# 30stomercury/Automatic-Speech-Recognition

Hardware: AMD Instinct MI355X
Metric: utterances/sec (train step) LibriSpeech-360 char-LAS @1/2/4/8 GPU; dev-clean WER (higher is better)
Workload: dtype bf16; 1 GPU; LibriSpeech-100 char LAS (BASELINE configs[1]): 3xpBLSTM-256 listener + 1xLSTM-512 speller, additive attention, MFCC-39, bucket B=48 T=1274, U=191, V=30; full train step fwd+bwd+clip+Adam; cell=lstm, per_gpu_batch=48, global_batch=48, frames=1274, dec_steps=191, parallelism=dp1, params=9679774

## Files before the change

automatic-speech-recognition_amd/csrc/las_common.h:

```cpp
#pragma once
#include <hip/hip_runtime.h>
#include <stdint.h>
#include <stddef.h>
#include "../../include/las_hip.h"

#if defined(__HIP_DEVICE_COMPILE__) && !defined(__gfx950__)
#error "liblas_hip.so is written for gfx950 (MI355X / CDNA4) only"
#endif

void las_set_error(const char* fmt, ...);
int las_device_cus();
int las_xcd_round_robin();

#define LAS_ARG(cond, ...)                                   \
    do { if (!(cond)) { las_set_error(__VA_ARGS__); return -1; } } while (0)
#define LAS_HIP(expr)                                        \
    do { hipError_t e__ = (expr);                            \
         if (e__ != hipSuccess) { las_set_error("%s -> %s", #expr, hipGetErrorString(e__)); \
                                  return (int)e__; } } while (0)
#ifdef LAS_DEBUG_SYNC
#define LAS_LAUNCHED()                                       \
    do { hipError_t e__ = hipGetLastError();                 \
         if (e__ == hipSuccess) e__ = hipDeviceSynchronize(); \
         if (e__ != hipSuccess) { las_set_error("%s:%d: launch failed: %s", __FILE__, __LINE__, hipGetErrorString(e__)); \
// ... 169 lines not shown
static inline int cdiv(long long a, long long b) { return (int)((a + b - 1) / b); }

extern "C" int las_colsum_dt(const void* X, int dtype, int rows, int cols, int ldx, float beta, float* out, void* ws,
                             size_t ws_bytes, void* stream);

size_t las_skinny_pack_bytes(int K, int N);
int las_skinny_pack(const float* W, int ldw, int K, int N, int transposed, void* packed, hipStream_t st);
int las_skinny_gemm(const float* A, int lda, int M, int K, const void* packed, int N, float* C, int ldc,
                    const float* bias, hipStream_t st);
int las_skinny_gemm_bf16(const unsigned short* A, int lda, int M, int K, const void* packed, int N, float* C, int ldc,
                         const float* bias, hipStream_t st);
int las_skinny_gemm_bf16_tanh(const unsigned short* A, int lda, int M, int K, const void* packed, int N, const float* bias, float* eh, int ldh,
                              unsigned short* b0, int ld0, unsigned short* b1, int ld1, hipStream_t st);
int las_skinny_gemm_bf16_tanh_bwd(const unsigned short* A, int lda, int M, int K, const void* packed, int N, float* C, int ldc, int c0, int D,
                                  const float* h, int ldh, const float* sa, int lda_, const float* sb, int ldb, int vlast, float* gp, int ldg,
                                  unsigned short* gb, int ldgb, hipStream_t st);
int las_skinny_gemm_bf16_lstm_bwd(const unsigned short* A, int lda, int M, int K, const void* packed, int N, float* C, int ldc, int c0, int D,
                                  const float* sa, int lda_, const float* sb, int ldb, int vlast, float* gp, int ldg, unsigned short* gb, int ldgb,
                                  const float* c, const float* cp, float* dC, int ldc_, hipStream_t st);
int las_skinny_lstm_bf16(const unsigned short* A, int lda, int M, int K, const void* packed, int D, const float* bias, float fb, const float* cprev,
                         float* c, float* h, float* gates, unsigned short* b0, int ld0, unsigned short* b1, int ld1, hipStream_t st);
bool las_skinny_ok(int M, int K, int N, int lda, const void* A);

typedef las_lstm_cell_args LstmCellLaunch;
int las_lstm_cell_rows_launch(const LstmCellLaunch& a, hipStream_t st);
int las_lstm_cell_check(const LstmCellLaunch& a);
int las_lstm_cell_rows_launch2(const LstmCellLaunch& a, const LstmCellLaunch& b, hipStream_t st);
```

automatic-speech-recognition_amd/csrc/speller.hip:

```cpp
#include "las_common.h"
#include "lstm_cell_rows.h"
#include <type_traits>
#include <math.h>

#define LAS_MAX_NL 4

constexpr int RNT = 1024;
constexpr int RNG = RNT / 32;
constexpr int RNW = RNT / 64;
constexpr int RNH = RNT / 128;

struct LoopProd {
    const u16x8_t* Bp; int KS, K, N, nct, M, pn, R;
    const float* bias;
    float* C; long long c_step; int ldc;
    unsigned long long* gA; int gA_row;
    unsigned long long* gC; int gC_row;
    unsigned long long* xcc;
    int nap;
    int budget;
    int* status;
};
#define LOOP_POLL_TIMEOUT(lp)                                                                                   \
    do { if ((lp).status) (lp).status[0] = LAS_SPELLER_STATUS_TIMEOUT; __builtin_amdgcn_s_waitcnt(0); __builtin_amdgcn_endpgm(); } while (0)
// ... 2578 lines not shown
}

__global__ __launch_bounds__(256) void dkeys_kernel(DecDev a, float* __restrict__ dKeys) {
    const int b = blockIdx.y, tt = blockIdx.x * 8 + (threadIdx.x >> 5), sl = threadIdx.x & 31;
    const int B = a.B, Tp = a.Tp, A = a.A, U = a.U;
    if (tt >= Tp) return;
    for (int a4 = sl; a4 < A / 4; a4 += 32) {
        const unsigned short* kr = a.keysbf + ((size_t)b * Tp + tt) * A + a4 * 4;
        const float k0 = bf2f(kr[0]), k1 = bf2f(kr[1]), k2 = bf2f(kr[2]), k3 = bf2f(kr[3]);
        float4 acc = make_float4(0.f, 0.f, 0.f, 0.f);
#pragma unroll 8
        for (int t = 0; t < U; ++t) {
            const float de = a.dE[((size_t)t * B + b) * Tp + tt];
            const float4 q4 = reinterpret_cast<const float4*>(a.Q + ((size_t)t * B + b) * A)[a4];
            const float v0 = tanh_fast(k0 + q4.x), v1 = tanh_fast(k1 + q4.y), v2 = tanh_fast(k2 + q4.z), v3 = tanh_fast(k3 + q4.w);
            acc.x = fmaf(de, 1.f - v0 * v0, acc.x); acc.y = fmaf(de, 1.f - v1 * v1, acc.y);
            acc.z = fmaf(de, 1.f - v2 * v2, acc.z); acc.w = fmaf(de, 1.f - v3 * v3, acc.w);
        }
        const float4 u4 = reinterpret_cast<const float4*>(a.u)[a4];
        float4* o = reinterpret_cast<float4*>(dKeys + ((size_t)b * Tp + tt) * A) + a4;
        float4 cur = *o;
        cur.x = fmaf(acc.x, u4.x, cur.x); cur.y = fmaf(acc.y, u4.y, cur.y); cur.z = fmaf(acc.z, u4.z, cur.z); cur.w = fmaf(acc.w, u4.w, cur.w);
        *o = cur;
    }
}

constexpr int EMB_MAX_V = 16384, EMB_MAX_N = 49152;
__global__ __launch_bounds__(1024) void emb_hist_kernel(const int* __restrict__ tok, int n, int V, int* __restrict__ start) {
    extern __shared__ int cnt[];
    int* part = cnt + V;
    const int tid = threadIdx.x;
    for (int v = tid; v < V; v += 1024) cnt[v] = 0;
    __syncthreads();
    for (int i = tid; i < n; i += 1024) { const int v = tok[i]; if (v >= 0 && v < V) atomicAdd(&cnt[v], 1); }
    __syncthreads();
    const int per = (V + 1023) / 1024, v0 = tid * per, v1 = min(V, v0 + per);
    int s_ = 0;
    for (int v = v0; v < v1; ++v) s_ += cnt[v];
    part[tid] = s_;
    __syncthreads();
    for (int off = 1; off < 1024; off <<= 1) {
        const int x = tid >= off ? part[tid - off] : 0;
        __syncthreads();
        part[tid] += x;
        __syncthreads();
    }
// ... 132 lines not shown
    w.fcS = o;    o += align256(C > 0 ? (size_t)U * B * Tp * C * f : 0);
    w.dfcS = o;   o += align256(C > 0 ? (size_t)U * B * Tp * C * f : 0);
    w.dlocwP = o; o += align256(C > 0 ? (size_t)B * DLW_SPLIT * Kc * C * f : 0);
    w.dlocbP = o; o += align256(C > 0 ? (size_t)B * DLW_SPLIT * C * f : 0);
    w.wide = o;   o += align256(wide_layout(B, Tp, A, D, NL, G, C).total);
    w.gemm = o;
    size_t big = (size_t)I0D * G * D;
    if ((size_t)D * V > big) big = (size_t)D * V;
    if ((size_t)8 * V * E > big) big = (size_t)8 * V * E;
    o += align256(big * 8 * f);
    w.total = o;
    return w;
}

static size_t act_save_f_offset(int U, int B, int Tp, int A) { return align256((size_t)LAS_ACT_HDR * 4 + (size_t)U * B * Tp * A * 2); }
extern "C" size_t las_speller_act_save_bytes(int U, int B, int Tp, int A, int C) {
    return act_save_f_offset(U, B, Tp, A) + (size_t)U * B * Tp * (C > 0 ? C : 0) * sizeof(float);
}
extern "C" size_t las_speller_workspace_bytes(int B, int Tp, int Hd, int A, int D, int NL, int E, int V, int U, int cell) {
    const int G = cell == LAS_CELL_LSTM ? 4 : 1;
    return bwd_layout(B, Tp, Hd, A, D, NL, E, V, U, G, 256, 16).total;
}

static int fill_dev(const las_speller_fwd_args* f, DecDev& d) {
    LAS_ARG(f, "speller: null args");
    LAS_ARG(f->B > 0 && f->Tp > 0 && f->Hd > 0 && f->A > 0 && f->D > 0 && f->E > 0 && f->V > 0 && f->U > 0,
            "speller: non-positive dimension");
    LAS_ARG(f->NL >= 1 && f->NL <= LAS_MAX_NL, "speller: NL=%d unsupported (1..%d)", f->NL, LAS_MAX_NL);
    LAS_ARG(f->D % 4 == 0 && f->Hd % 4 == 0, "speller: D and Hd must be multiples of 4");
    LAS_ARG(f->A % 4 == 0 && f->A <= 256, "speller: attention size must be a multiple of 4 and <= 256 (got %d)", f->A);
    LAS_ARG(f->cell == LAS_CELL_RNN || f->cell == LAS_CELL_LSTM, "speller: bad cell");
    LAS_ARG(f->mode == LAS_ATT_ADD || f->mode == LAS_ATT_LOC, "speller: bad attention mode");
    LAS_ARG(f->mode == LAS_ATT_ADD || (f->loc_w && f->loc_b && f->Wf && f->Kc > 0 && f->Kc <= 256 && f->C > 0 && f->C <= 16),
            "speller: location-aware attention needs loc_w/loc_b/Wf, Kc<=256, C<=16");
    LAS_ARG(f->enc && f->keys && f->enc_len && f->Ws && f->u && f->emb && f->Wv && f->bv && f->cellW && f->cellb,
            "speller: null parameter pointer");
    LAS_ARG(f->tokens_in && f->logits && f->alphas && f->hs && f->gates && f->xin0, "speller: null buffer pointer");
    LAS_ARG(f->cell == LAS_CELL_RNN || f->cs, "speller: lstm needs cs");
    LAS_ARG(!f->step_logits || f->tokens_out, "speller: step_logits needs tokens_out");
    LAS_ARG((((uintptr_t)f->keys | (uintptr_t)f->u | (uintptr_t)f->Ws) & 15) == 0, "speller: keys/u/Ws must be 16-byte aligned");
    d.B = f->B; d.Tp = f->Tp; d.Hd = f->Hd; d.A = f->A; d.D = f->D; d.NL = f->NL; d.E = f->E; d.V = f->V; d.U = f->U;
    d.mode = f->mode; d.Kc = f->mode == LAS_ATT_LOC ? f->Kc : 0; d.C = f->mode == LAS_ATT_LOC ? f->C : 0;
    d.step_logits = f->step_logits; d.flags = f->flags; d.fb = f->forget_bias; d.seed = f->seed;
    d.row_group = (f->row_group > 0 && f->B % f->row_group == 0) ? f->row_group : 0;
    d.shared_ops = ((f->flags & LAS_SPELLER_SHARED_OPERANDS) && d.row_group > 0) ? 1 : 0;
    LAS_ARG(!(f->flags & LAS_SPELLER_SHARED_OPERANDS) || d.row_group > 0, "speller: LAS_SPELLER_SHARED_OPERANDS needs row_group > 0 with B %% row_group == 0");
// ... 161 lines not shown
                if (int rc = f->companion ? las_lstm_cell_rows_launch2(c, *f->companion, st) : las_lstm_cell_rows_launch(c, st)) return rc;
                break;
            }
            if (skinny) {
                GEMM_OK(las_skinny_gemm_bf16(d.xbf, I0D, B, I0D, packF, GD, d.gates + ((size_t)0 * U + t) * B * GD, GD, f->cellb[0], st));
            } else {
                const bool hw = f->ws && f->ws_bytes > wl_.gemm;
                GEMM_OK(las_gemm(f->prec, 0, 0, B, GD, I0D, 1.f, d.xin0 + (size_t)t * B * I0D, I0D, 0, f->cellW[0], GD, 0, 0.f,
                                 d.gates + ((size_t)0 * U + t) * B * GD, GD, 0, f->cellb[0], LAS_ACT_NONE, 1, 0, 0,
                                 hw ? (char*)f->ws + wl_.gemm : nullptr, hw ? f->ws_bytes - wl_.gemm : 0, st));
            }
            for (int l = 1; l < NL; ++l) {
                hipLaunchKernelGGL((dec_pointwise_fwd_kernel<CELL, FAST>), dim3(B), dim3(256), 0, st, d, l - 1, t);
                LAS_LAUNCHED();
                float* gl = d.gates + ((size_t)l * U + t) * B * GD;
                GEMM_OK(las_gemm(f->prec, 0, 0, B, GD, D, 1.f, d.hs + ((size_t)(l - 1) * (U + 1) + t + 1) * B * D, D, 0,
                                 f->cellW[l], GD, 0, 0.f, gl, GD, 0, f->cellb[l], LAS_ACT_NONE, 1, 0, 0, nullptr, 0, st));
                GEMM_OK(las_gemm(f->prec, 0, 0, B, GD, D, 1.f, d.hs + ((size_t)l * (U + 1) + t) * B * D, D, 0,
                                 f->cellW[l] + (size_t)D * GD, GD, 0, 1.f, gl, GD, 0, nullptr, LAS_ACT_NONE, 1, 0, 0, nullptr, 0, st));
            }
        }
    }
    if (d.step_logits != 1) {
        GEMM_OK(las_gemm(f->prec, 0, 0, U * B, V, D, 1.f, d.hs + ((size_t)(NL - 1) * (U + 1) + 1) * B * D, D, 0, d.Wv, V, 0,
                         0.f, d.logits, V, 0, d.bv, LAS_ACT_NONE, 1, 0, 0, nullptr, 0, st));
    }
    return 0;
}

extern "C" int las_speller_fwd(const las_speller_fwd_args* f, void* stream) {
    DecDev d;
    if (int rc = fill_dev(f, d)) return rc;
    hipStream_t st = (hipStream_t)stream;
    const bool fast = f->prec == LAS_PREC_BF16;
    if (f->cell == LAS_CELL_LSTM)
        return fast ? speller_fwd_impl<LAS_CELL_LSTM, true>(f, d, st) : speller_fwd_impl<LAS_CELL_LSTM, false>(f, d, st);
    return fast ? speller_fwd_impl<LAS_CELL_RNN, true>(f, d, st) : speller_fwd_impl<LAS_CELL_RNN, false>(f, d, st);
}

template <int CELL, bool FAST>
static int speller_bwd_impl(const las_speller_bwd_args* bk, DecDev d, int part, hipStream_t st) {
    constexpr int G = CELL == LAS_CELL_LSTM ? 4 : 1;
    const las_speller_fwd_args* f = &bk->f;
    const int B = d.B, D = d.D, NL = d.NL, U = d.U, E = d.E, Hd = d.Hd, V = d.V, A = d.A, Tp = d.Tp;
    const int GD = G * D, I0D = E + Hd + D, TOP = NL - 1, prec = f->prec;
    const bool loc = d.mode == LAS_ATT_LOC;
    const BwdWs w = bwd_layout(B, Tp, Hd, A, D, NL, E, V, U, G, d.Kc, d.C);
    LAS_ARG(f->ws && f->ws_bytes >= w.total, "las_speller_bwd: workspace too small (%zu < %zu)", f->ws_bytes, w.total);
// ... 12 lines not shown
    if (p.lds_row > 64 * 1024) LAS_LDS_ATTR((dec_step_bwd_kernel<CELL, FAST, true>), 150 * 1024);
    const bool skinny = p.skinny, wide = p.family == LAS_SPELLER_RAN_WIDE, loop = p.family == LAS_SPELLER_RAN_LOOP;
    void* packB = base + w.packB;
    if (skinny) d.dgbf = (unsigned short*)(base + w.dgbf);
    if (p.family != LAS_SPELLER_RAN_F32_ROWS) {
        if ((part & 1) && p.bf_copies) GEMM_OK(make_bf_copies(d, base, w, st));
        d.dE = (float*)(base + w.dE);
    }
    if (part & 1) g_last_variant[1] = p.ran;
    if (p.act_save && bk->f.act_save) {
        d.actS = (unsigned*)bk->f.act_save;
        if (d.mode == LAS_ATT_LOC) d.fcSave = (float*)((char*)bk->f.act_save + act_save_f_offset(U, B, Tp, A));
    }
    if (skinny && (part & 1)) {
        if (loop) GEMM_OK(las_skinny_pack(f->cellW[0] + (size_t)E * GD, GD, GD, Hd + D, 1, packB, st));
        else      GEMM_OK(las_skinny_pack(f->cellW[0], GD, GD, I0D, 1, packB, st));
    }
    if (part & 1) {
    d.rec[0] = d.dXin0; d.recLd[0] = I0D; d.recOff[0] = E + Hd;
    for (int l = 1; l < NL; ++l) { d.rec[l] = tmp + (size_t)l * B * 2 * D; d.recLd[l] = 2 * D; d.recOff[l] = D; }

    LAS_HIP(hipMemsetAsync(base + w.dH, 0, w.dXin0 - w.dH, st));
    LAS_HIP(hipMemsetAsync(base + w.duRows, 0, w.dV - w.duRows, st));
    GEMM_OK(las_gemm(prec, 0, 1, U * B, D, V, 1.f, bk->dlogits, V, 0, d.Wv, V, 0, 0.f, dHl, D, 0, nullptr, LAS_ACT_NONE, 1, 0, 0,
                     nullptr, 0, st));
    for (int l = 0; l < NL; ++l)
        GEMM_OK(las_gemm(prec, 0, 0, U * B, A, D, 1.f, d.hs + (size_t)l * (U + 1) * B * D, D, 0, d.Ws + (size_t)l * D * A, A, 0,
                         l ? 1.f : 0.f, d.Q, A, 0, nullptr, LAS_ACT_NONE, 1, 0, 0, nullptr, 0, st));

    switch (p.family) {
    case LAS_SPELLER_RAN_LOOP:
        loop_prod_dims(d.lp, B, Hd + D, GD);
        d.lp.Bp = reinterpret_cast<const u16x8_t*>(packB); d.lp.bias = nullptr;
        d.lp.C = d.dXin0 + E; d.lp.c_step = (long long)B * I0D; d.lp.ldc = I0D;
        d.lp.gA = (unsigned long long*)(base + w.granG); d.lp.gA_row = GD / 4;
        d.lp.gC = (unsigned long long*)(base + w.granB); d.lp.gC_row = (Hd + D) / 2;
        d.lp.xcc = (unsigned long long*)(base + w.xccs);
        LAS_HIP(hipMemsetAsync(base + w.granG, 0, w.xccs + 256 * 8 - w.granG, st));
        GEMM_OK(with_ne(Tp, [&](auto ne) {
            constexpr int NE = decltype(ne)::value;
            if (p.locloop) LAS_LDS_LAUNCH((dec_loop_bwd_kernel<CELL, NE, true>), dim3(8 * (d.lp.pn + d.lp.R)), dim3(RNT), p.lds_loop, LOOP_LDS_MAX, st, d);
            else           LAS_LDS_LAUNCH((dec_loop_bwd_kernel<CELL, NE, false>), dim3(8 * (d.lp.pn + d.lp.R)), dim3(RNT), p.lds_loop, LOOP_LDS_MAX, st, d);
            return 0;
        }));
        break;
    case LAS_SPELLER_RAN_WIDE:
        GEMM_OK((wide_bwd_steps<CELL, FAST>(bk, d, w, base, packB, dHl, tmp, gws, gws_bytes, st)));
        break;
// ... 18 lines not shown
            if (t < 0) break;
            for (int l = TOP; l >= 0; --l) {
                const float* dG = d.gates + ((size_t)l * U + t) * B * GD;
                if (l == 0 && skinny) {
                    GEMM_OK(las_skinny_gemm_bf16(d.dgbf, GD, B, GD, packB, I0D, d.dXin0 + (size_t)t * B * I0D, I0D, nullptr, st));
                } else if (l == 0) {
                    GEMM_OK(las_gemm(prec, 0, 1, B, I0D, GD, 1.f, dG, GD, 0, f->cellW[0], GD, 0, 0.f, d.dXin0 + (size_t)t * B * I0D,
                                     I0D, 0, nullptr, LAS_ACT_NONE, 1, 0, 0, gws, gws_bytes, st));
                } else {
                    float* tl = tmp + (size_t)l * B * 2 * D;
                    GEMM_OK(las_gemm(prec, 0, 1, B, 2 * D, GD, 1.f, dG, GD, 0, f->cellW[l], GD, 0, 0.f, tl, 2 * D, 0, nullptr,
                                     LAS_ACT_NONE, 1, 0, 0, nullptr, 0, st));
                    hipLaunchKernelGGL((dec_pointwise_bwd_kernel<CELL, FAST>), dim3(B), dim3(256), 0, st, d, l - 1, t, (const float*)tl, 2 * D);
                    LAS_LAUNCHED();
                }
            }
        }
    }

    if (p.locloop) {
        hipLaunchKernelGGL(dkeys_loc_kernel, dim3(cdiv(Tp, 8), B), dim3(256), 0, st, d, bk->d_keys);
        LAS_LAUNCHED();
    } else if (!wide && p.family != LAS_SPELLER_RAN_F32_ROWS) {
        hipLaunchKernelGGL(dkeys_kernel, dim3(cdiv(Tp, 8), B), dim3(256), 0, st, d, bk->d_keys);
        LAS_LAUNCHED();
    }
    GEMM_OK(las_gemm(prec, 1, 0, Tp, Hd, U, 1.f, d.alphas, B * Tp, Tp, d.dXin0 + E, B * I0D, I0D, 1.f, bk->d_enc, Hd,
                     (long long)Tp * Hd, nullptr, LAS_ACT_NONE, B, 0, 0, nullptr, 0, st));
    }
    if (!(part & 2)) return 0;
    const int UB = U * B;
    GEMM_OK(las_gemm(prec, 1, 0, I0D, GD, UB, 1.f, d.xin0, I0D, 0, d.gates, GD, 0, 1.f, bk->dcellW[0], GD, 0, nullptr,
                     LAS_ACT_NONE, 1, 0, 0, gws, gws_bytes, st));
    for (int l = 0; l < NL; ++l) {
        const float* dG = d.gates + (size_t)l * U * B * GD;
        GEMM_OK(las_colsum(dG, UB, GD, GD, 1.f, bk->dcellb[l], gws, gws_bytes, st));
        if (l > 0) {
            GEMM_OK(las_gemm(prec, 1, 0, D, GD, UB, 1.f, d.hs + ((size_t)(l - 1) * (U + 1) + 1) * B * D, D, 0, dG, GD, 0, 1.f,
                             bk->dcellW[l], GD, 0, nullptr, LAS_ACT_NONE, 1, 0, 0, gws, gws_bytes, st));
            GEMM_OK(las_gemm(prec, 1, 0, D, GD, UB, 1.f, d.hs + (size_t)l * (U + 1) * B * D, D, 0, dG, GD, 0, 1.f,
                             bk->dcellW[l] + (size_t)D * GD, GD, 0, nullptr, LAS_ACT_NONE, 1, 0, 0, gws, gws_bytes, st));
        }
        GEMM_OK(las_gemm(prec, 1, 0, D, A, UB, 1.f, d.hs + (size_t)l * (U + 1) * B * D, D, 0, d.dQ, A, 0, 1.f,
                         bk->dWs + (size_t)l * D * A, A, 0, nullptr, LAS_ACT_NONE, 1, 0, 0, gws, gws_bytes, st));
    }
    GEMM_OK(las_gemm(prec, 1, 0, D, V, UB, 1.f, d.hs + ((size_t)TOP * (U + 1) + 1) * B * D, D, 0, bk->dlogits, V, 0, 1.f,
                     bk->dWv, V, 0, nullptr, LAS_ACT_NONE, 1, 0, 0, gws, gws_bytes, st));
// ... 70 lines not shown
```

automatic-speech-recognition_amd/las/_hip.py:

```python
import collections
import ctypes
import os
from ctypes import (POINTER, Structure, c_char_p, c_double, c_float, c_int, c_longlong, c_size_t,
                    c_void_p)

import torch

PREC_F32, PREC_BF16 = 0, 1
CELL_RNN, CELL_LSTM = 0, 1
ACT_NONE, ACT_TANH = 0, 1
ATT_ADD, ATT_LOC = 0, 1
DT_F32, DT_BF16 = 0, 1

_HERE = os.path.dirname(os.path.abspath(__file__))
LIB_PATH = os.environ.get("LAS_LIB_PATH") or os.path.join(os.path.dirname(_HERE), "lib", "liblas_hip.so")
_lib = None


class LstmCellArgs(Structure):
    _fields_ = [("x", c_void_p), ("x_bf16", c_int), ("ldx", c_int), ("I", c_int), ("ids", c_void_p), ("id_shift", c_int), ("xrows", c_void_p),
                ("h", c_void_p), ("ldh", c_int), ("Wx", c_void_p), ("Wh", c_void_p), ("bias", c_void_p), ("c_prev", c_void_p), ("fb", c_float),
                ("c_out", c_void_p), ("h_out", c_void_p), ("gates_out", c_void_p), ("M", c_int), ("H", c_int), ("fast", c_int),
                ("h_bf16", c_int), ("h_out_bf16", c_void_p)]

# ... 96 lines not shown
    "las_gemm_dt": (c_int, [c_int, c_int, c_int, c_int, c_int, c_int, c_float, c_void_p, c_int, c_longlong,
                            c_void_p, c_int, c_longlong, c_int, c_float, c_void_p, c_int, c_longlong, c_void_p, c_int,
                            c_int, c_int, c_int, c_void_p, c_size_t, c_void_p]),
    "las_gemm_workspace_bytes": (c_size_t, [c_int, c_int, c_int, c_int, c_int]),
    "las_wgrad_ih_hh_workspace_bytes": (c_size_t, [c_int, c_int, c_int, c_int, c_int, c_int]),
    "las_wgrad_ih_hh": (c_int, [c_void_p, c_void_p, c_int, c_int, c_void_p, c_int, c_longlong, c_void_p, c_int, c_int, c_int, c_int, c_int, c_int,
                                c_void_p, c_void_p, c_void_p, c_size_t, c_void_p]),
    "las_gemm_kk": (c_int, [c_int, c_int, c_int, c_void_p, c_longlong, c_void_p, c_longlong, c_void_p, c_int, c_longlong,
                            c_void_p, c_int, c_void_p]),
    "las_gemm_kk_tanhgrad": (c_int, [c_int, c_int, c_int, c_void_p, c_longlong, c_void_p, c_longlong, c_void_p, c_int, c_longlong,
                            c_void_p, c_int, c_void_p, c_longlong, c_void_p]),
    "las_colsum_workspace_bytes": (c_size_t, [c_int]),
    "las_colsum": (c_int, [c_void_p, c_int, c_int, c_int, c_float, c_void_p, c_void_p, c_size_t, c_void_p]),
    "las_tanh_bwd": (c_int, [c_void_p, c_int, c_void_p, c_int, c_void_p, c_int, c_int, c_int, c_void_p]),
    "las_rnn_seq_workspace_bytes": (c_size_t, [c_int, c_int, c_int, c_int]),
    "las_rnn_seq_io_dtype": (c_int, [c_int, c_int, c_int]),
    "las_rnn_seq_plan": (c_int, [c_int, c_int, c_int, c_int, c_int, c_int, c_int, POINTER(RnnSeqPlanInfo)]),
    "las_rnn_seq_fwd": (c_int, [POINTER(RnnSeqArgs), c_void_p]),
    "las_rnn_seq_bwd": (c_int, [POINTER(RnnSeqArgs), c_void_p]),
    "las_colsum_dt": (c_int, [c_void_p, c_int, c_int, c_int, c_int, c_float, c_void_p, c_void_p, c_size_t, c_void_p]),
    "las_tanh_bwd_dt": (c_int, [c_void_p, c_int, c_int, c_void_p, c_int, c_int, c_void_p, c_int, c_int, c_int, c_int, c_void_p]),
    "las_speller_workspace_bytes": (c_size_t, [c_int] * 10),
    "las_speller_act_save_bytes": (c_size_t, [c_int] * 5),
    "las_speller_fwd": (c_int, [POINTER(SpellerFwdArgs), c_void_p]),
    "las_speller_bwd": (c_int, [POINTER(SpellerBwdArgs), c_void_p]),
    "las_speller_bwd_part": (c_int, [POINTER(SpellerBwdArgs), c_int, c_void_p]),
    "las_speller_last_variant": (c_int, [c_int]),
    "las_bn_workspace_bytes": (c_size_t, [c_longlong, c_int]),
    "las_bn_relu_fwd": (c_int, [c_void_p, c_longlong, c_int, c_void_p, c_void_p, c_float, c_void_p, c_void_p, c_void_p, c_void_p, c_float, c_int,
                                c_void_p, c_void_p, c_size_t, c_void_p]),
    "las_bn_relu_bwd": (c_int, [c_void_p, c_void_p, c_void_p, c_longlong, c_int, c_void_p, c_void_p, c_void_p, c_int, c_void_p, c_void_p, c_void_p,
                                c_void_p, c_size_t, c_void_p]),
    "las_dropout_pair_fwd": (c_int, [c_void_p, c_int, c_longlong, c_int, c_int, c_void_p, c_void_p, c_int, c_int, c_float, ctypes.c_ulonglong, c_void_p]),
    "las_dropout_pair_bwd": (c_int, [c_void_p, c_void_p, c_int, c_int, c_longlong, c_int, c_void_p, c_int, c_int, c_float, ctypes.c_ulonglong, c_void_p]),
    "las_ce_loss_workspace_bytes": (c_size_t, [c_int, c_int]),
    "las_ce_loss": (c_int, [c_void_p, c_longlong, c_longlong, c_void_p, c_int, c_int, c_int, c_int, c_float, c_int,
                            c_void_p, c_void_p, c_void_p, c_void_p, c_size_t, c_void_p]),
    "las_ctc_workspace_bytes": (c_size_t, [c_int, c_int, c_int]),
    "las_ctc_loss": (c_int, [c_void_p, c_longlong, c_longlong, c_int, c_void_p, c_int, c_int, c_void_p, c_int, c_int, c_int,
                             c_void_p, c_void_p, c_void_p, c_void_p, c_int, c_longlong, c_longlong, c_void_p, c_size_t, c_void_p]),
    "las_ctc_log_softmax": (c_int, [c_void_p, c_int, c_int, c_int, c_void_p, c_void_p]),
    "las_ctc_prefix_step": (c_int, [c_void_p, c_void_p, c_int, c_int, c_int, c_int, c_int, c_void_p, c_void_p, c_float, c_void_p,
                                    c_void_p, c_int, c_void_p, c_void_p, c_void_p, c_void_p, c_void_p, c_int, c_void_p]),
    "las_ctc_align_workspace_bytes": (c_size_t, [c_int, c_int, c_int]),
    "las_ctc_align": (c_int, [c_void_p, c_int, c_int, c_void_p, c_int, c_void_p, c_int, c_void_p, c_int, c_void_p, c_void_p, c_void_p,
                              c_void_p, c_void_p, c_size_t, c_void_p]),
# ... 378 lines not shown
    def __init__(self, name):
        self.name = name

    def __enter__(self):
        if ROCTX:
            torch.cuda.nvtx.range_push(self.name)
        if _PROF is not None:
            self.e0 = torch.cuda.Event(enable_timing=True)
            self.e1 = torch.cuda.Event(enable_timing=True)
            self.e0.record()
        return self

    def __exit__(self, *exc):
        if _PROF is not None:
            self.e1.record()
            _PROF.setdefault(self.name, []).append((self.e0, self.e1))
        if ROCTX:
            torch.cuda.nvtx.range_pop()
        return False


SEQ_AGENT_GRANULES, SEQ_NO_KSPLIT, SEQ_NO_HELPER_WAVES, SEQ_ROWS16, SEQ_NO_WARMERS, SEQ_F32_VALU, SEQ_PREPARED = 1, 2, 4, 8, 16, 32, 64
SPELLER_NO_PF_ROWS, SPELLER_NO_BF_ROWS, SPELLER_NO_FUSED_STEP, SPELLER_REUSE_PREP, SPELLER_NO_LOGITS, SPELLER_ROWS_SHARE4 = 1, 2, 4, 8, 16, 32
SPELLER_WIDE, SPELLER_NO_WIDE, SPELLER_SHARED_OPERANDS = 64, 128, 1 << 14
SEQ_STATUS = {1: "forward sweep: a cluster partner did not publish h within the spin bound (or a chunk of the x-projection did not "
                 "complete while the sweep was waiting for it: kernels of different streams must be able to overlap -- under a "
                 "tool that serialises kernels, e.g. rocprofv3 --pmc, set LAS_ALLOW_SERIAL_STREAMS=1)",
              2: "BPTT sweep: a cluster partner did not publish its partial dh within the spin bound",
              3: "Speller loop kernel: a partner workgroup was not seen within the poll bound (the one-launch decode loop needs one "
                 "workgroup per compute unit co-resident; on a shared / partitioned device set LAS_NO_FUSED_STEP=1)"}


def seq_p(p):
    return (int(p) & 0xf) << 8


def speller_spin_log2(n):
    return (int(n) & 0x1f) << 8


def seq_spin_log2(n):
    return (int(n) & 0x1f) << 16


def _flags_from_env():
    e = os.environ.get
    f = (SEQ_AGENT_GRANULES if e("LAS_AGENT_GRANULES") == "1" else 0) | (SEQ_NO_KSPLIT if e("LAS_NO_KSPLIT") else 0) | \
        (SEQ_NO_HELPER_WAVES if e("LAS_NO_HELPER_WAVES") else 0) | (SEQ_ROWS16 if e("LAS_ROWS16") else 0) | \
        (SEQ_NO_WARMERS if e("LAS_NO_WARMERS") else 0) | (SEQ_F32_VALU if e("LAS_F32_VALU") else 0)
    if e("LAS_SEQ_P"):
        f |= seq_p(e("LAS_SEQ_P"))
    if e("LAS_SPIN_LOG2"):
        f |= seq_spin_log2(e("LAS_SPIN_LOG2"))
    g = (SPELLER_NO_PF_ROWS if e("LAS_NO_PF_ROWS") == "1" else 0) | (SPELLER_NO_BF_ROWS if e("LAS_NO_BF_ROWS") == "1" else 0) | \
        (SPELLER_NO_FUSED_STEP if e("LAS_NO_FUSED_STEP") == "1" else 0) | (SPELLER_WIDE if e("LAS_SPELLER_WIDE") == "1" else 0) | \
        (SPELLER_NO_WIDE if e("LAS_NO_WIDE") == "1" else 0)
    return f, g


seq_flags, speller_flags = _flags_from_env()

_status = {}


def _devkey(dev):
    d = torch.device(dev) if not isinstance(dev, torch.device) else dev
    if d.type == "cuda" and d.index is None:
        d = torch.device("cuda", torch.cuda.current_device())
    return str(d)


def status_word(dev):
    key = _devkey(dev)
    t = _status.get(key)
    if t is None:
        t = torch.zeros(2, dtype=torch.int32, device=dev)
        _status[key] = t
    return t

# ... 245 lines not shown
```

include/las_hip.h:

```cpp
#ifndef LAS_HIP_H
#define LAS_HIP_H

#include <stddef.h>

#ifdef __cplusplus
extern "C" {
#endif

enum { LAS_PREC_F32 = 0, LAS_PREC_BF16 = 1 };
enum { LAS_CELL_RNN = 0, LAS_CELL_LSTM = 1 };
enum { LAS_ACT_NONE = 0, LAS_ACT_TANH = 1 };
enum { LAS_ATT_ADD = 0, LAS_ATT_LOC = 1 };
enum { LAS_DT_F32 = 0, LAS_DT_BF16 = 1 };

#define LAS_HIP_ABI_VERSION 605
int         las_version(void);
const char* las_last_error(void);

int las_gemm(int prec, int transA, int transB, int M, int N, int K,
             float alpha, const float* A, int lda, long long strideA,
             const float* B, int ldb, long long strideB,
             float beta, float* C, int ldc, long long strideC,
             const float* bias, int act, int batch,
             int a_mask_period, int a_mask_skip, void* ws, size_t ws_bytes, void* stream);
// ... 81 lines not shown
    const void* dout; int ld_dout; long long dout_bstride;
    float* dbias_fw; float* dbias_bw;
    const int* dout_chunk_flag; int dout_chunk_rows, dout_rows;
    int* progress; int progress_steps;
} las_rnn_seq_args;
int las_rnn_seq_fwd(const las_rnn_seq_args* a, void* stream);
int las_rnn_seq_bwd(const las_rnn_seq_args* a, void* stream);

int las_gemm_kk_frames(int nb, int T, int lo0, int nlo, int hi0, int nhi, int N, int K, const void* A, long long lda,
                       const void* B, long long ldb, void* C, int c_dtype, long long ldc, const float* bias, int act,
                       const void* y_tanh, long long ldy, void* stream);
int las_set_word(int* word, int value, void* stream);

enum { LAS_SPELLER_STATUS_TIMEOUT = 3 };
enum { LAS_SPELLER_NO_PF_ROWS = 1,
       LAS_SPELLER_NO_BF_ROWS = 2,
       LAS_SPELLER_NO_FUSED_STEP = 4,
       LAS_SPELLER_REUSE_PREP = 8 };
enum { LAS_SPELLER_NO_LOGITS = 16 };
enum { LAS_SPELLER_ROWS_SHARE4 = 32 };
enum { LAS_SPELLER_WIDE = 64,
       LAS_SPELLER_NO_WIDE = 128,
       LAS_SPELLER_SHARED_OPERANDS = 1 << 14 };
#define LAS_SPELLER_SPIN_LOG2(n) (((n) & 31) << 8)
typedef struct {
    int B, Tp, Hd, A, D, NL, E, V, U, cell, mode, prec, Kc, C, step_logits, keep_state0;
    int flags;
    float forget_bias;
    unsigned long long seed;
    const float *enc, *keys; const int* enc_len;
    const float *Ws, *u, *emb, *Wv, *bv, *loc_w, *loc_b, *Wf;
    const float* const* cellW; const float* const* cellb;
    int* tokens_in; int* tokens_out;
    float *logits, *alphas;
    const float* align0;
    const float* emb_mask;
    const float* emb_noise;
    float *hs, *cs, *gates, *xin0;
    void* act_save;
    void* ws; size_t ws_bytes;
    int* status;
    const struct las_lstm_cell_args* companion;
    const struct las_lstm_cell_args* companion_rows;
    int row_group;
} las_speller_fwd_args;
size_t las_speller_workspace_bytes(int B, int Tp, int Hd, int A, int D, int NL, int E, int V, int U, int cell);
size_t las_speller_act_save_bytes(int U, int B, int Tp, int A, int C);
int las_speller_fwd(const las_speller_fwd_args* a, void* stream);

typedef struct {
    las_speller_fwd_args f;
    const float* dlogits;
    float *d_enc, *d_keys, *dWs, *du, *demb, *dWv, *dbv, *dloc_w, *dloc_b, *dWf;
    float* const* dcellW; float* const* dcellb;
} las_speller_bwd_args;
int las_speller_bwd(const las_speller_bwd_args* a, void* stream);
int las_speller_bwd_part(const las_speller_bwd_args* a, int part, void* stream);
enum { LAS_SPELLER_RAN_LOOP = 1,
       LAS_SPELLER_RAN_PF_ROWS = 2,
       LAS_SPELLER_RAN_BF_ROWS = 4,
       LAS_SPELLER_RAN_F32_ROWS = 8,
       LAS_SPELLER_RAN_SKINNY = 16,
       LAS_SPELLER_RAN_LOC = 32,
       LAS_SPELLER_RAN_UPPER_SKINNY = 64,
       LAS_SPELLER_RAN_WIDE = 128 };
int las_speller_last_variant(int which);

size_t las_ce_loss_workspace_bytes(int B, int U);
int las_ce_loss(const float* logits, long long sb, long long st, const int* y, int ldy,
                int B, int U, int V, float epsilon, int smooth,
// ... 172 lines not shown
```

Before: 3529 utterances/s.

## Add small-vocab MFMA output head kernels and LDS-tiled attention dKeys backward

Adds dedicated kernels for the output projection when the vocabulary is tiny (V<=64). They stage Wv in LDS as bf16 MFMA fragments, for both the forward logits and the backward dH. These replace the generic las_gemm on the fused-loop path. The dKeys backward is also replaced with an LDS-tiled kernel: it stages Q and dE chunks in shared memory with register prefetch and splits the time loop across waves, with a final reduction. The aim is to cut generic GEMM overhead and redundant global loads in the attention-key gradient, at the cost of bf16 rounding in the head and extra code paths behind env flags.

Measured after the change: 3548 utterances/s (median of 6 runs). Within noise of the previous version (+0.5%).

```diff
diff --git a/automatic-speech-recognition_amd/csrc/las_common.h b/automatic-speech-recognition_amd/csrc/las_common.h
--- a/automatic-speech-recognition_amd/csrc/las_common.h
+++ b/automatic-speech-recognition_amd/csrc/las_common.h
@@ -215,6 +215,10 @@
                          float* c, float* h, float* gates, unsigned short* b0, int ld0, unsigned short* b1, int ld1, hipStream_t st);
 bool las_skinny_ok(int M, int K, int N, int lda, const void* A);
 
+bool las_head_small_v_ok(int M, int D, int V, const void* H, const void* dH);
+int las_head_logits(const float* H, const float* Wv, const float* bv, float* out, int M, int D, int V, hipStream_t st);
+int las_head_dh(const float* dL, const float* Wv, float* out, int M, int D, int V, hipStream_t st);
+
 typedef las_lstm_cell_args LstmCellLaunch;
 int las_lstm_cell_rows_launch(const LstmCellLaunch& a, hipStream_t st);
 int las_lstm_cell_check(const LstmCellLaunch& a);
diff --git a/automatic-speech-recognition_amd/csrc/speller.hip b/automatic-speech-recognition_amd/csrc/speller.hip
--- a/automatic-speech-recognition_amd/csrc/speller.hip
+++ b/automatic-speech-recognition_amd/csrc/speller.hip
@@ -2624,6 +2624,82 @@
         float4 cur = *o;
         cur.x = fmaf(acc.x, u4.x, cur.x); cur.y = fmaf(acc.y, u4.y, cur.y); cur.z = fmaf(acc.z, u4.z, cur.z); cur.w = fmaf(acc.w, u4.w, cur.w);
         *o = cur;
+    }
+}
+
+constexpr int DK_FB = 8, DK_TS = 32, DK_AC = 128;
+__device__ __forceinline__ void dkeys_fetch(const DecDev& a, const int b, const int tt0, const int a0, const int t0, const int tid,
+                                            float4 (&pq)[4], float& pde) {
+#pragma unroll
+    for (int j = 0; j < 4; ++j) {
+        const int idx = tid + 256 * j, t = t0 + (idx >> 5), col = a0 + (idx & 31) * 4;
+        pq[j] = (t < a.U && col < a.A) ? *reinterpret_cast<const float4*>(a.Q + ((size_t)t * a.B + b) * a.A + col) : make_float4(0.f, 0.f, 0.f, 0.f);
+    }
+    const int t = t0 + (tid >> 3), tt = tt0 + (tid & 7);
+    pde = (t < a.U && tt < a.Tp) ? a.dE[((size_t)t * a.B + b) * a.Tp + tt] : 0.f;
+}
+__global__ __launch_bounds__(256, 4) void dkeys_lds_kernel(DecDev a, float* __restrict__ dKeys) {
+    __shared__ __attribute__((aligned(16))) float Qs[DK_TS * DK_AC];
+    __shared__ __attribute__((aligned(16))) float dEs[DK_TS * DK_FB];
+    static_assert(4 * DK_FB * DK_AC <= DK_TS * DK_AC, "the partial sums reuse Qs");
+    const int b = blockIdx.y, tt0 = blockIdx.x * DK_FB, tid = threadIdx.x, wv = tid >> 6, fh = (tid >> 5) & 1, sl = tid & 31;
+    const int Tp = a.Tp, A = a.A, U = a.U;
+    for (int a0 = 0; a0 < A; a0 += DK_AC) {
+        const int ac = a0 + sl * 4;
+        float k[4][4], acc[4][4];
+#pragma unroll
+        for (int f = 0; f < 4; ++f) {
+            const int tt = tt0 + fh * 4 + f;
+            uint2 kb = make_uint2(0u, 0u);
+            if (tt < Tp && ac < A) kb = *reinterpret_cast<const uint2*>(a.keysbf + ((size_t)b * Tp + tt) * A + ac);
+            k[f][0] = bf2f((unsigned short)(kb.x & 0xffffu)); k[f][1] = bf2f((unsigned short)(kb.x >> 16));
+            k[f][2] = bf2f((unsigned short)(kb.y & 0xffffu)); k[f][3] = bf2f((unsigned short)(kb.y >> 16));
+#pragma unroll
+            for (int c = 0; c < 4; ++c) acc[f][c] = 0.f;
+        }
+        float4 pq[4];
+        float pde;
+        dkeys_fetch(a, b, tt0, a0, 0, tid, pq, pde);
+        for (int t0 = 0; t0 < U; t0 += DK_TS) {
+            __syncthreads();
+#pragma unroll
+            for (int j = 0; j < 4; ++j) reinterpret_cast<float4*>(Qs)[tid + 256 * j] = pq[j];
+            dEs[tid] = pde;
+            __syncthreads();
+            if (t0 + DK_TS < U) dkeys_fetch(a, b, tt0, a0, t0 + DK_TS, tid, pq, pde);
+#pragma unroll 2
+            for (int s = 0; s < DK_TS / 4; ++s) {
+                const int ts = wv * (DK_TS / 4) + s;
+                if (t0 + ts >= U) break;
+                const float4 q4 = *reinterpret_cast<const float4*>(Qs + ts * DK_AC + sl * 4);
+                const float4 d4 = *reinterpret_cast<const float4*>(dEs + ts * DK_FB + fh * 4);
+                const float de[4] = {d4.x, d4.y, d4.z, d4.w};
+#pragma unroll
+                for (int f = 0; f < 4; ++f) {
+                    const float v0 = tanh_fast(k[f][0] + q4.x), v1 = tanh_fast(k[f][1] + q4.y), v2 = tanh_fast(k[f][2] + q4.z), v3 = tanh_fast(k[f][3] + q4.w);
+                    acc[f][0] = fmaf(de[f], 1.f - v0 * v0, acc[f][0]); acc[f][1] = fmaf(de[f], 1.f - v1 * v1, acc[f][1]);
+                    acc[f][2] = fmaf(de[f], 1.f - v2 * v2, acc[f][2]); acc[f][3] = fmaf(de[f], 1.f - v3 * v3, acc[f][3]);
+                }
+            }
+        }
+        __syncthreads();
+#pragma unroll
+        for (int f = 0; f < 4; ++f)
+            *reinterpret_cast<float4*>(Qs + ((wv * DK_FB + fh * 4 + f) * DK_AC) + sl * 4) = make_float4(acc[f][0], acc[f][1], acc[f][2], acc[f][3]);
+        __syncthreads();
+        const int tt = tt0 + (tid >> 5);
+        if (tt < Tp && ac < A) {
+            const float* pp = Qs + (tid >> 5) * DK_AC + sl * 4;
+            const float4 p0 = *reinterpret_cast<const float4*>(pp), p1 = *reinterpret_cast<const float4*>(pp + DK_FB * DK_AC);
+            const float4 p2 = *reinterpret_cast<const float4*>(pp + 2 * DK_FB * DK_AC), p3 = *reinterpret_cast<const float4*>(pp + 3 * DK_FB * DK_AC);
+            const float4 s4 = make_float4(((p0.x + p1.x) + p2.x) + p3.x, ((p0.y + p1.y) + p2.y) + p3.y, ((p0.z + p1.z) + p2.z) + p3.z,
+                                          ((p0.w + p1.w) + p2.w) + p3.w);
+            const float4 u4 = *reinterpret_cast<const float4*>(a.u + ac);
+            float4* o = reinterpret_cast<float4*>(dKeys + ((size_t)b * Tp + tt) * A + ac);
+            float4 cur = *o;
+            cur.x = fmaf(s4.x, u4.x, cur.x); cur.y = fmaf(s4.y, u4.y, cur.y); cur.z = fmaf(s4.z, u4.z, cur.z); cur.w = fmaf(s4.w, u4.w, cur.w);
+            *o = cur;
+        }
     }
 }
 
@@ -2802,6 +2878,16 @@
     return bwd_layout(B, Tp, Hd, A, D, NL, E, V, U, G, 256, 16).total;
 }
 
+extern "C" size_t las_speller_workspace_offset(int B, int Tp, int Hd, int A, int D, int NL, int E, int V, int U, int cell, int region) {
+    const BwdWs w = bwd_layout(B, Tp, Hd, A, D, NL, E, V, U, cell == LAS_CELL_LSTM ? 4 : 1, 256, 16);
+    switch (region) {
+    case LAS_SPELLER_WS_KEYS_BF16: return w.keysbf;
+    case LAS_SPELLER_WS_DE:        return w.dE;
+    case LAS_SPELLER_WS_Q:         return w.Q;
+    default:                       return (size_t)-1;
+    }
+}
+
 static int fill_dev(const las_speller_fwd_args* f, DecDev& d) {
     LAS_ARG(f, "speller: null args");
     LAS_ARG(f->B > 0 && f->Tp > 0 && f->Hd > 0 && f->A > 0 && f->D > 0 && f->E > 0 && f->V > 0 && f->U > 0,
@@ -3009,8 +3095,11 @@
         }
     }
     if (d.step_logits != 1) {
-        GEMM_OK(las_gemm(f->prec, 0, 0, U * B, V, D, 1.f, d.hs + ((size_t)(NL - 1) * (U + 1) + 1) * B * D, D, 0, d.Wv, V, 0,
-                         0.f, d.logits, V, 0, d.bv, LAS_ACT_NONE, 1, 0, 0, nullptr, 0, st));
+        const float* htop = d.hs + ((size_t)(NL - 1) * (U + 1) + 1) * B * D;
+        if (FAST && p.family == LAS_SPELLER_RAN_LOOP && !p.locloop && !(d.flags & LAS_SPELLER_NO_SMALL_V) && las_head_small_v_ok(U * B, D, V, htop, nullptr))
+            GEMM_OK(las_head_logits(htop, d.Wv, d.bv, d.logits, U * B, D, V, st));
+        else
+            GEMM_OK(las_gemm(f->prec, 0, 0, U * B, V, D, 1.f, htop, D, 0, d.Wv, V, 0, 0.f, d.logits, V, 0, d.bv, LAS_ACT_NONE, 1, 0, 0, nullptr, 0, st));
     }
     return 0;
 }
@@ -3069,8 +3158,11 @@
 
     LAS_HIP(hipMemsetAsync(base + w.dH, 0, w.dXin0 - w.dH, st));
     LAS_HIP(hipMemsetAsync(base + w.duRows, 0, w.dV - w.duRows, st));
-    GEMM_OK(las_gemm(prec, 0, 1, U * B, D, V, 1.f, bk->dlogits, V, 0, d.Wv, V, 0, 0.f, dHl, D, 0, nullptr, LAS_ACT_NONE, 1, 0, 0,
-                     nullptr, 0, st));
+    if (FAST && loop && !p.locloop && !(d.flags & LAS_SPELLER_NO_SMALL_V) && las_head_small_v_ok(U * B, D, V, nullptr, dHl))
+        GEMM_OK(las_head_dh(bk->dlogits, d.Wv, dHl, U * B, D, V, st));
+    else
+        GEMM_OK(las_gemm(prec, 0, 1, U * B, D, V, 1.f, bk->dlogits, V, 0, d.Wv, V, 0, 0.f, dHl, D, 0, nullptr, LAS_ACT_NONE, 1, 0, 0,
+                         nullptr, 0, st));
     for (int l = 0; l < NL; ++l)
         GEMM_OK(las_gemm(prec, 0, 0, U * B, A, D, 1.f, d.hs + (size_t)l * (U + 1) * B * D, D, 0, d.Ws + (size_t)l * D * A, A, 0,
                          l ? 1.f : 0.f, d.Q, A, 0, nullptr, LAS_ACT_NONE, 1, 0, 0, nullptr, 0, st));
@@ -3135,7 +3227,8 @@
         hipLaunchKernelGGL(dkeys_loc_kernel, dim3(cdiv(Tp, 8), B), dim3(256), 0, st, d, bk->d_keys);
         LAS_LAUNCHED();
     } else if (!wide && p.family != LAS_SPELLER_RAN_F32_ROWS) {
-        hipLaunchKernelGGL(dkeys_kernel, dim3(cdiv(Tp, 8), B), dim3(256), 0, st, d, bk->d_keys);
+        if (!loop || (d.flags & LAS_SPELLER_DKEYS_STEPWISE)) hipLaunchKernelGGL(dkeys_kernel, dim3(cdiv(Tp, 8), B), dim3(256), 0, st, d, bk->d_keys);
+        else                                                 hipLaunchKernelGGL(dkeys_lds_kernel, dim3(cdiv(Tp, DK_FB), B), dim3(256), 0, st, d, bk->d_keys);
         LAS_LAUNCHED();
     }
     GEMM_OK(las_gemm(prec, 1, 0, Tp, Hd, U, 1.f, d.alphas, B * Tp, Tp, d.dXin0 + E, B * I0D, I0D, 1.f, bk->d_enc, Hd,
diff --git a/automatic-speech-recognition_amd/csrc/speller_head.hip b/automatic-speech-recognition_amd/csrc/speller_head.hip
--- /dev/null
+++ b/automatic-speech-recognition_amd/csrc/speller_head.hip
@@ -0,0 +1,153 @@
+#include "las_common.h"
+
+typedef unsigned int hd_u32x4_t __attribute__((ext_vector_type(4)));
+
+constexpr int HEAD_MAX_V = 64;
+constexpr int HEAD_LDS_MAX = 64 * 1024;
+constexpr int HEAD_STAGE = 4, HEAD_KB = 8;
+
+template <int NCT>
+__global__ __launch_bounds__(256) void head_logits_kernel(const float* __restrict__ H, const float* __restrict__ Wv, const float* __restrict__ bv,
+                                                          float* __restrict__ out, int M, int D, int V) {
+    extern __shared__ __attribute__((aligned(16))) unsigned short head_lds[];
+    u16x8_t* wfrag = reinterpret_cast<u16x8_t*>(head_lds);
+    const int tid = threadIdx.x, lane = tid & 63, wv = tid >> 6;
+    const int KS = D >> 5;
+    for (int e0 = tid; e0 < KS * NCT * 64; e0 += 256 * HEAD_STAGE) {
+        float x[HEAD_STAGE][8];
+#pragma unroll
+        for (int i = 0; i < HEAD_STAGE; ++i) {
+            const int e = min(e0 + 256 * i, KS * NCT * 64 - 1);
+            const int l = e & 63, ct = (e >> 6) % NCT, ks = (e >> 6) / NCT;
+            const int v = ct * 16 + (l & 15), d0 = ks * 32 + (l >> 4) * 8;
+#pragma unroll
+            for (int j = 0; j < 8; ++j) {
+                const float w = Wv[(size_t)(d0 + j) * V + min(v, V - 1)];
+                x[i][j] = v < V ? w : 0.f;
+            }
+        }
+#pragma unroll
+        for (int i = 0; i < HEAD_STAGE; ++i) {
+            u16x8_t f;
+#pragma unroll
+            for (int j = 0; j < 8; ++j) f[j] = f2bf(x[i][j]);
+            if (e0 + 256 * i < KS * NCT * 64) wfrag[e0 + 256 * i] = f;
+        }
+    }
+    __syncthreads();
+    const int row0 = (blockIdx.x * 4 + wv) * 16;
+    if (row0 >= M) return;
+    const int r = min(row0 + (lane & 15), M - 1);
+    const float4* hp = reinterpret_cast<const float4*>(H + (size_t)r * D + (lane >> 4) * 8);
+    f32x4_t acc[NCT];
+#pragma unroll
+    for (int ct = 0; ct < NCT; ++ct) acc[ct] = (f32x4_t){0.f, 0.f, 0.f, 0.f};
+    for (int ks0 = 0; ks0 < KS; ks0 += HEAD_KB) {
+        float4 a0[HEAD_KB], a1[HEAD_KB];
+#pragma unroll
+        for (int i = 0; i < HEAD_KB; ++i) {
+            const int ks = min(ks0 + i, KS - 1);
+            a0[i] = hp[ks * 8]; a1[i] = hp[ks * 8 + 1];
+        }
+#pragma unroll
+        for (int i = 0; i < HEAD_KB; ++i) {
+            const int ks = min(ks0 + i, KS - 1);
+            const hd_u32x4_t pk = {f2bf2(a0[i].x, a0[i].y), f2bf2(a0[i].z, a0[i].w), f2bf2(a1[i].x, a1[i].y), f2bf2(a1[i].z, a1[i].w)};
+            const u16x8_t Af = __builtin_bit_cast(u16x8_t, ks0 + i < KS ? pk : (hd_u32x4_t){0u, 0u, 0u, 0u});
+#pragma unroll
+            for (int ct = 0; ct < NCT; ++ct) acc[ct] = mfma_bf16_16x16x32(Af, wfrag[(ks * NCT + ct) * 64 + lane], acc[ct]);
+        }
+    }
+#pragma unroll
+    for (int ct = 0; ct < NCT; ++ct) {
+        const int col = ct * 16 + (lane & 15);
+        if (col >= V) continue;
+        const float bias = bv ? bv[col] : 0.f;
+#pragma unroll
+        for (int i = 0; i < 4; ++i) {
+            const int row = row0 + (lane >> 4) * 4 + i;
+            if (row < M) out[(size_t)row * V + col] = acc[ct][i] + bias;
+        }
+    }
+}
+
+template <int KS>
+__global__ __launch_bounds__(256) void head_dh_kernel(const float* __restrict__ dL, const float* __restrict__ Wv, float* __restrict__ out,
+                                                      int M, int D, int V) {
+    extern __shared__ __attribute__((aligned(16))) unsigned short head_lds[];
+    u16x8_t* wfrag = reinterpret_cast<u16x8_t*>(head_lds);
+    const int tid = threadIdx.x, lane = tid & 63, wv = tid >> 6;
+    const int NDT = D >> 4;
+    for (int e0 = tid; e0 < NDT * KS * 64; e0 += 256 * HEAD_STAGE) {
+        float x[HEAD_STAGE][8];
+#pragma unroll
+        for (int i = 0; i < HEAD_STAGE; ++i) {
+            const int e = min(e0 + 256 * i, NDT * KS * 64 - 1);
+            const int l = e & 63, ks = (e >> 6) % KS, dt = (e >> 6) / KS;
+            const int d = dt * 16 + (l & 15), v0 = ks * 32 + (l >> 4) * 8;
+#pragma unroll
+            for (int j = 0; j < 8; ++j) {
+                const float w = Wv[(size_t)d * V + min(v0 + j, V - 1)];
+                x[i][j] = v0 + j < V ? w : 0.f;
+            }
+        }
+#pragma unroll
+        for (int i = 0; i < HEAD_STAGE; ++i) {
+            u16x8_t f;
+#pragma unroll
+            for (int j = 0; j < 8; ++j) f[j] = f2bf(x[i][j]);
+            if (e0 + 256 * i < NDT * KS * 64) wfrag[e0 + 256 * i] = f;
+        }
+    }
+    __syncthreads();
+    const int row0 = (blockIdx.x * 2 + (wv & 1)) * 16;
+    if (row0 >= M) return;
+    const int row = row0 + (lane & 15);
+    const float* lp = dL + (size_t)min(row, M - 1) * V;
+    u16x8_t Bf[KS];
+#pragma unroll
+    for (int ks = 0; ks < KS; ++ks) {
+        const int v0 = ks * 32 + (lane >> 4) * 8;
+#pragma unroll
+        for (int j = 0; j < 8; ++j)
+            Bf[ks][j] = f2bf(lp[min(v0 + j, V - 1)] * (v0 + j < V ? 1.f : 0.f));
+    }
+    const int dt0 = (wv >> 1) * (NDT >> 1), dt1 = dt0 + (NDT >> 1);
+    for (int dt = dt0; dt < dt1; ++dt) {
+        f32x4_t acc = {0.f, 0.f, 0.f, 0.f};
+#pragma unroll
+        for (int ks = 0; ks < KS; ++ks) acc = mfma_bf16_16x16x32(wfrag[(dt * KS + ks) * 64 + lane], Bf[ks], acc);
+        if (row < M) *reinterpret_cast<float4*>(out + (size_t)row * D + dt * 16 + (lane >> 4) * 4) = make_float4(acc[0], acc[1], acc[2], acc[3]);
+    }
+}
+
+bool las_head_small_v_ok(int M, int D, int V, const void* H, const void* dH) {
+    return M > 0 && V > 0 && V <= HEAD_MAX_V && D > 0 && (D % 32) == 0 && (size_t)D * cdiv(V, 16) * 32 <= (size_t)HEAD_LDS_MAX &&
+           (size_t)D * cdiv(V, 32) * 64 <= (size_t)HEAD_LDS_MAX && (((uintptr_t)H | (uintptr_t)dH) & 15) == 0;
+}
+
+int las_head_logits(const float* H, const float* Wv, const float* bv, float* out, int M, int D, int V, hipStream_t st) {
+    LAS_ARG(las_head_small_v_ok(M, D, V, H, nullptr), "las_head_logits: M=%d D=%d V=%d is not served", M, D, V);
+    const int nct = cdiv(V, 16);
+    const size_t lds = (size_t)D * nct * 32;
+    const dim3 grid(cdiv(M, 64)), block(256);
+    switch (nct) {
+    case 1:  hipLaunchKernelGGL(head_logits_kernel<1>, grid, block, lds, st, H, Wv, bv, out, M, D, V); break;
+    case 2:  hipLaunchKernelGGL(head_logits_kernel<2>, grid, block, lds, st, H, Wv, bv, out, M, D, V); break;
+    case 3:  hipLaunchKernelGGL(head_logits_kernel<3>, grid, block, lds, st, H, Wv, bv, out, M, D, V); break;
+    default: hipLaunchKernelGGL(head_logits_kernel<4>, grid, block, lds, st, H, Wv, bv, out, M, D, V); break;
+    }
+    LAS_LAUNCHED();
+    return 0;
+}
+
+int las_head_dh(const float* dL, const float* Wv, float* out, int M, int D, int V, hipStream_t st) {
+    LAS_ARG(las_head_small_v_ok(M, D, V, nullptr, out), "las_head_dh: M=%d D=%d V=%d is not served", M, D, V);
+    const int ks = cdiv(V, 32);
+    const size_t lds = (size_t)D * ks * 64;
+    const dim3 grid(cdiv(M, 32)), block(256);
+    if (ks == 1) hipLaunchKernelGGL(head_dh_kernel<1>, grid, block, lds, st, dL, Wv, out, M, D, V);
+    else         hipLaunchKernelGGL(head_dh_kernel<2>, grid, block, lds, st, dL, Wv, out, M, D, V);
+    LAS_LAUNCHED();
+    return 0;
+}
diff --git a/automatic-speech-recognition_amd/las/_hip.py b/automatic-speech-recognition_amd/las/_hip.py
--- a/automatic-speech-recognition_amd/las/_hip.py
+++ b/automatic-speech-recognition_amd/las/_hip.py
@@ -142,6 +142,7 @@
     "las_tanh_bwd_dt": (c_int, [c_void_p, c_int, c_int, c_void_p, c_int, c_int, c_void_p, c_int, c_int, c_int, c_int, c_void_p]),
     "las_speller_workspace_bytes": (c_size_t, [c_int] * 10),
     "las_speller_act_save_bytes": (c_size_t, [c_int] * 5),
+    "las_speller_workspace_offset": (c_size_t, [c_int] * 11),
     "las_speller_fwd": (c_int, [POINTER(SpellerFwdArgs), c_void_p]),
     "las_speller_bwd": (c_int, [POINTER(SpellerBwdArgs), c_void_p]),
     "las_speller_bwd_part": (c_int, [POINTER(SpellerBwdArgs), c_int, c_void_p]),
@@ -566,6 +567,7 @@
 
 SEQ_AGENT_GRANULES, SEQ_NO_KSPLIT, SEQ_NO_HELPER_WAVES, SEQ_ROWS16, SEQ_NO_WARMERS, SEQ_F32_VALU, SEQ_PREPARED = 1, 2, 4, 8, 16, 32, 64
 SPELLER_NO_PF_ROWS, SPELLER_NO_BF_ROWS, SPELLER_NO_FUSED_STEP, SPELLER_REUSE_PREP, SPELLER_NO_LOGITS, SPELLER_ROWS_SHARE4 = 1, 2, 4, 8, 16, 32
+SPELLER_NO_SMALL_V, SPELLER_DKEYS_STEPWISE = 1 << 15, 1 << 16
 SPELLER_WIDE, SPELLER_NO_WIDE, SPELLER_SHARED_OPERANDS = 64, 128, 1 << 14
 SEQ_STATUS = {1: "forward sweep: a cluster partner did not publish h within the spin bound (or a chunk of the x-projection did not "
                  "complete while the sweep was waiting for it: kernels of different streams must be able to overlap -- under a "
@@ -598,7 +600,8 @@
         f |= seq_spin_log2(e("LAS_SPIN_LOG2"))
     g = (SPELLER_NO_PF_ROWS if e("LAS_NO_PF_ROWS") == "1" else 0) | (SPELLER_NO_BF_ROWS if e("LAS_NO_BF_ROWS") == "1" else 0) | \
         (SPELLER_NO_FUSED_STEP if e("LAS_NO_FUSED_STEP") == "1" else 0) | (SPELLER_WIDE if e("LAS_SPELLER_WIDE") == "1" else 0) | \
-        (SPELLER_NO_WIDE if e("LAS_NO_WIDE") == "1" else 0)
+        (SPELLER_NO_WIDE if e("LAS_NO_WIDE") == "1" else 0) | (SPELLER_NO_SMALL_V if e("LAS_SPELLER_SMALL_V") == "0" else 0) | \
+        (SPELLER_DKEYS_STEPWISE if e("LAS_DKEYS_OLD") == "1" else 0)
     return f, g
 
 
diff --git a/include/las_hip.h b/include/las_hip.h
--- a/include/las_hip.h
+++ b/include/las_hip.h
@@ -127,6 +127,8 @@
 enum { LAS_SPELLER_WIDE = 64,
        LAS_SPELLER_NO_WIDE = 128,
        LAS_SPELLER_SHARED_OPERANDS = 1 << 14 };
+enum { LAS_SPELLER_NO_SMALL_V = 1 << 15,
+       LAS_SPELLER_DKEYS_STEPWISE = 1 << 16 };
 #define LAS_SPELLER_SPIN_LOG2(n) (((n) & 31) << 8)
 typedef struct {
     int B, Tp, Hd, A, D, NL, E, V, U, cell, mode, prec, Kc, C, step_logits, keep_state0;
@@ -151,6 +153,8 @@
 } las_speller_fwd_args;
 size_t las_speller_workspace_bytes(int B, int Tp, int Hd, int A, int D, int NL, int E, int V, int U, int cell);
 size_t las_speller_act_save_bytes(int U, int B, int Tp, int A, int C);
+enum { LAS_SPELLER_WS_KEYS_BF16 = 0, LAS_SPELLER_WS_DE = 1, LAS_SPELLER_WS_Q = 2 };
+size_t las_speller_workspace_offset(int B, int Tp, int Hd, int A, int D, int NL, int E, int V, int U, int cell, int region);
 int las_speller_fwd(const las_speller_fwd_args* a, void* stream);
 
 typedef struct {
```
